# matthieugomez/LeastSquaresOptim.jl

Hardware: AMD Instinct MI355X
Metric: lm_lsmr_outer_iterations_per_sec (higher is better)
Workload: dtype f64

## Files before the change

leastsquaresoptim.jl_amd/csrc/lsq_optimize.hip:

```cpp
#include <chrono>
#include <cmath>
#include <cstring>

#include "lsq_solver.h"
#include "lsq_spmv.h"

static constexpr double MIN_DELTA = 1e-16, MAX_DELTA = 1e16, MIN_STEP_QUALITY = 1e-3;
static constexpr double MIN_DIAGONAL = 1e-6, MAX_DIAGONAL = 1e32;
static constexpr double DECREASE_THRESHOLD = 0.25, INCREASE_THRESHOLD = 0.75;

enum { SL_GRAD = 8, SL_DX = 9, SL_NONFIN = 10, SL_TRIAL = 11, SL_PRED = 12, SL_SSR = 13, SL_W0 = 14, SL_W1 = 15,
       SL_W2 = 16, SL_SUM = 17 };

extern "C" int lsq_solver_create(lsq_ctx *c, lsq_mat *J, int kind, int for_lm, lsq_solver **out) {
    LSQ_RANGE("lsq_solver_create");
    if (!c || !J || !out) return LSQ_EARG;
    if (kind == LSQ_QR && J->kind != LSQ_MAT_DENSE) {
        lsq_set_error("solver QR() is not available for sparse Jacobians. Choose between Cholesky() and LSMR()");
        return LSQ_EARG;
    }
    const bool blockdiag = kind == LSQ_CHOLESKY && J->kind == LSQ_MAT_CSC && J->bd_blocks > 0;
    const bool bordered = kind == LSQ_CHOLESKY && J->kind == LSQ_MAT_CSC && J->br_blocks > 0;
    if (kind == LSQ_CHOLESKY && J->kind != LSQ_MAT_DENSE && !blockdiag && !bordered) {
        lsq_set_error("MethodError: no AbstractAllocatedSolver for Cholesky() with a sparse Jacobian "
// ... 377 lines not shown
    }
}

static inline int ngrid(const lsq_ctx *c, long long n) {
    long long g = (n + LSQ_NT - 1) / LSQ_NT;
    long long cap = (long long)c->num_cus * 8;
    if (g > cap) g = cap;
    return g < 1 ? 1 : (int)g;
}

static int sumsq_to_slot(lsq_ctx *c, bool exact, long long n, const double *x, int ctr, double *d_out,
                         LsqSlotPublish pub = LsqSlotPublish()) {
    if (exact) return lsq_seq_reduce(c, 1, (int)n, x, nullptr, nullptr, d_out);
    long long g = (n + LSQ_NT - 1) / LSQ_NT, cap = (long long)c->num_cus * 2;
    if (g > cap) g = cap;
    if (g < 1) g = 1;
    LSQ_LAUNCH(k_sumsq_slot, dim3((int)g), dim3(LSQ_NT), 0, c->stream, n, x, c->d_partials, lsq_ctr(c, ctr), d_out,
                       pub);
    return LSQ_OK;
}
static int model_f(double *out, const double *x, void *user);
static int model_g(lsq_mat *J, const double *x, void *user);
static int model_f_sumsq(void *user, double *out, const double *x, int ctr, double *d_out, LsqSlotPublish pub, bool *done,
                         const int *skip = nullptr);
struct SpecGrad {
    int *gate;
    double ssr;
    double *grad;
    bool launched;
};
static int model_pair_tail(void *user, lsq_mat *J, const double *dx, const double *fcur, double *ftrial, const double *xt,
                           double *slot_pred, double *slot_trial, LsqSlotPublish pub, const int *skip, bool *done,
                           SpecGrad *sg = nullptr);
static void model_trial_buffers(void *user, const double *xt, double **t_out, double **s_out);
static int f_then_sumsq(lsq_ctx *c, bool exact, lsq_f_callback f, void *user, long long m, double *out, const double *x, int ctr,
                        double *d_out, LsqSlotPublish pub = LsqSlotPublish(), const int *skip = nullptr) {
    if (!exact && f == model_f) {
        bool fused = false;
        if (model_f_sumsq(user, out, x, ctr, d_out, pub, &fused, skip) != 0) {
            lsq_set_error("user callback reported failure");
            return LSQ_ECALLBACK;
        }
        if (fused) return LSQ_OK;
    } else if (f(out, x, user) != 0) {
        lsq_set_error("user callback reported failure");
        return LSQ_ECALLBACK;
    }
    return sumsq_to_slot(c, exact, m, out, ctr, d_out, pub);
}
static int predicted_to_slot(lsq_ctx *c, bool exact, lsq_mat *J, const double *d, const double *f, double *scratch,
                             int ctr, double *d_out, LsqSlotPublish pub = LsqSlotPublish(), const int *skip = nullptr);
static int wdot_to_slot(lsq_ctx *c, bool exact, int n, const double *x, const double *y, const double *w, int ctr,
                        double *d_out);
static int gradient_into(lsq_ctx *c, bool exact, lsq_mat *J, const double *f, double *g);

struct LoopBuffers {
    lsq_ctx *c;
    int m, n;
    double *dx = nullptr, *dtd = nullptr, *xt = nullptr, *ftrial = nullptr;
    double *dgn = nullptr, *dgr = nullptr, *grad = nullptr, *fpred = nullptr;
    double *lo = nullptr, *hi = nullptr;
    int *gate_ring = nullptr;
// ... 174 lines not shown
            return LSQ_ECALLBACK;                         \
        }                                                 \
    } while (0)

static int call_g(lsq_g_callback g, lsq_mat *J, const double *x, void *user) {
    J->version++;
    if (J->kind == LSQ_MAT_CSC && !J->d_cs_user) J->csr_fresh = false;
    CB(g(J, x, user));
    return lsq_ensure_csr(J);
}
int lsq_call_g(lsq_g_callback g, lsq_mat *J, const double *x, void *user) { return call_g(g, J, x, user); }

struct IterateGuard {
    lsq_ctx *c;
    double *&x, *&fcur;
    double *x_user, *fcur_user;
    int m, n;
    ~IterateGuard() {
        if (x != x_user) lsq_d2d(c, x_user, x, (size_t)n * sizeof(double));
        if (fcur != fcur_user) lsq_d2d(c, fcur_user, fcur, (size_t)m * sizeof(double));
    }
};

static int start_residual(lsq_ctx *c, lsq_mat *J, lsq_f_callback f, void *user, double *fcur, const double *x, double *ssr,
                          int *nonfinite_at) {
    const int m = J->m, n = J->n;
    if (lsq_small_mat(J) || lsq_small_vec(m) || m <= 0) {
        CB(f(fcur, x, user));
        LSQ_TRY(lsq_sumsq(c, m, fcur, ssr));
        return lsq_first_nonfinite(c, n, x, nonfinite_at);
    }
    static_assert(SL_TRIAL == SL_NONFIN + 1, "the two scalars of the loop head travel together");
    LSQ_TRY(lsq_first_nonfinite_to_slot(c, n, x, c->d_slots + SL_NONFIN));
    LSQ_TRY(f_then_sumsq(c, false, f, user, m, fcur, x, 7, c->d_slots + SL_TRIAL));
    double sl[2];
    LSQ_TRY(lsq_read_slots(c, SL_NONFIN, 2, sl));
    *nonfinite_at = (int)sl[0];
    *ssr = sl[1];
    return LSQ_OK;
}

static int optimize_lm_loop(lsq_ctx *c, lsq_solver *sv, LoopBuffers &b, lsq_mat *J, double *x_user, double *fcur_user,
                            lsq_f_callback f, lsq_g_callback g, void *user, const lsq_options *o, lsq_result *r);
static int optimize_lm(lsq_ctx *c, lsq_solver *sv, LoopBuffers &b, lsq_mat *J, double *x_user, double *fcur_user,
                       lsq_f_callback f, lsq_g_callback g, void *user, const lsq_options *o, lsq_result *r) {
    ShardedExit ex{c, o};
    return ex.finish(optimize_lm_loop(c, sv, b, J, x_user, fcur_user, f, g, user, o, r));
}
static int optimize_lm_loop(lsq_ctx *c, lsq_solver *sv, LoopBuffers &b, lsq_mat *J, double *x_user, double *fcur_user,
                            lsq_f_callback f, lsq_g_callback g, void *user, const lsq_options *o, lsq_result *r) {
    const int m = J->m, n = J->n;
    double *x = x_user, *fcur = fcur_user, *xt = b.xt, *ftrial = b.ftrial;
    IterateGuard guard{c, x, fcur, x_user, fcur_user, m, n};
    double delta = o->delta > 0 ? o->delta : 10.0;
    double decrease_factor = 2.0;
    int f_calls = 0, g_calls = 0, mul_calls = 0, xc = 0, fc = 0, gc = 0;
    bool converged = false;
    double ssr;
    int iter = 0, nonfinite_at = -1;
    const bool sharded = o->row_allreduce != nullptr;
    if (sharded) CB(f(fcur, x, user));
    else LSQ_TRY(start_residual(c, J, f, user, fcur, x, &ssr, &nonfinite_at));
    f_calls++;
    auto rows_sum = [&](double *d_buf, int count) -> int {
        if (o->row_allreduce(d_buf, count, (void *)c->stream, o->row_allreduce_user) != 0) {
            lsq_set_error("row all-reduce callback reported failure");
            return LSQ_ECALLBACK;
        }
        return LSQ_OK;
    };
    if (sharded) {
        LSQ_TRY(sumsq_to_slot(c, false, m, fcur, 7, c->d_slots + SL_TRIAL));
        LSQ_TRY(rows_sum(c->d_slots + SL_TRIAL, 1));
        LSQ_TRY(lsq_read_slots(c, SL_TRIAL, 1, &ssr));
        LSQ_TRY(lsq_first_nonfinite(c, n, x, &nonfinite_at));
    }
    r->ssr0 = ssr;
    double maxabs_gr = INFINITY;
    bool need_jac = true;
    const int gn = ngrid(c, n);
    const bool exact = lsq_small_mat(J) && !sharded && !(sv->kind == LSQ_LSMR && sv->gen_ldiv);
    int last_inner = 0;
    const bool no_spec_grad = getenv("LSQ_NO_SPEC_GRADIENT") != nullptr;
    bool spec_launched = false, spec_grad_ready = false, spec_pending = false;
    struct SpecGuard { lsq_mat *J; bool &ready; bool &pending; ~SpecGuard() { if (ready || pending) lsq_sparse_colsum_forget(J); } }
        spec_guard{J, spec_grad_ready, spec_pending};
    int local_done = 0;
    double gssr = ssr, ggr = maxabs_gr;
    long long inner_total = 0;
    while (iter < o->iterations) {
        if (!o->allreduce && converged) break;
        if (o->allreduce && converged) {
            int all = 1;
            gssr = ssr; ggr = maxabs_gr;
            LSQ_TRY(global_exchange(o, &gssr, &ggr, &all));
            if (all) break;
            ++iter; local_done = 1;
            continue;
        }
        iter++;
        if (nonfinite_at >= 0) {
            r->bad_index = nonfinite_at;
            r->iterations = iter - 1;
            lsq_set_error("IsFiniteException: non-finite x at index %d", nonfinite_at);
            return LSQ_ENONFINITE;
        }
        if (need_jac) {
            LSQ_TRY(call_g(g, J, x, user));
            g_calls++;
            need_jac = false;
        }
        bool have_grad = false;
        if (spec_grad_ready) {
            lsq_sparse_grad_colsum_adopt(J);
            have_grad = true;
            spec_grad_ready = false;
        }
        const bool spec_ok = !no_spec_grad && !exact && !sharded && sv->kind == LSQ_LSMR && f == model_f && g == model_g &&
                             iter < o->iterations && !lsq_dbg_serial;
        spec_launched = false;
        if (!exact && J->colsum_version != J->version && lsq_can_fuse_grad_colsum(J)) {
            LSQ_TRY(lsq_sparse_grad_colsum(J, fcur, b.grad));
            have_grad = true;
        }
        const double *cs = nullptr;
        LSQ_TRY(lsq_rowshard_colsum(sv, J, &cs));
        const bool one_wg = !exact && n <= LSQ_ONE_WG_N;
        const bool lm_prep = one_wg && sv->kind == LSQ_LSMR && ssr >= 0.0 && lsq_lsmr_takes_lm_prep(sv, J);
        if (exact) LSQ_TRY(lsq_exact_lm_damp(c, n, cs, 1.0 / delta, b.dtd));
        else if (!one_wg) LSQ_LAUNCH(k_lm_damp, dim3(1), dim3(1024), 0, c->stream, n, cs, 1.0 / delta, b.dtd);
        {
            if (!have_grad) LSQ_TRY(gradient_into(c, exact, J, fcur, b.grad));
            if (sharded) LSQ_TRY(rows_sum(b.grad, n));
            if (lm_prep) {}
            else if (one_wg)
// ... 1 lines not shown
                                   x, b.lo, b.hi, c->d_slots + SL_GRAD);
            else
                LSQ_LAUNCH(k_gradnorm, dim3(gn), dim3(LSQ_NT), 0, c->stream, n, b.grad, x, b.lo, b.hi,
                                   c->d_partials, lsq_ctr(c, 4), c->d_slots + SL_GRAD);
            mul_calls++;
        }
        struct Xchg { const lsq_options *o; double *gssr, *ggr; } xchg{o, &gssr, &ggr};
        if (o->allreduce) {
            gssr = ssr; ggr = maxabs_gr;
            c->idle_hook = [](void *p) -> int {
                Xchg *q = (Xchg *)p;
                int all = 0;
                return global_exchange(q->o, q->gssr, q->ggr, &all);
            };
            c->idle_user = &xchg;
            c->idle_status = 0;
            if (sv->kind != LSQ_LSMR || exact) lsq_run_idle_hook(c);
        }
        int lmiter = 0;
        struct TailCtx {
            lsq_ctx *c; lsq_mat *J; LoopBuffers *b; lsq_f_callback f; void *user;
            const double *x, *fcur; double *xt, *ftrial;
            int m, n, gn; bool is_model; LsqSlotPublish pub; int launched;
            bool want_spec; double ssr; bool spec_launched; bool *spec_pending;
        } tc{c, J, &b, f, user, x, fcur, xt, ftrial, m, n, gn, !exact && f == model_f, LsqSlotPublish(), 0, spec_ok, ssr, false,
             &spec_pending};
        auto tail_fn = [](const int *skip, void *u) -> int {
            TailCtx &t = *(TailCtx *)u;
            lsq_ctx *c = t.c;
            double *t_out = nullptr, *s_out = nullptr;
            if (t.is_model) model_trial_buffers(t.user, t.xt, &t_out, &s_out);
            LSQ_LAUNCH(k_step, dim3(t.gn), dim3(LSQ_NT), 0, c->stream, t.n, t.x, t.b->dx, t.xt, c->d_partials,
                               lsq_ctr(c, 5), c->d_slots + SL_DX, c->d_slots + SL_NONFIN, t_out, s_out, skip);
            LSQ_HIP(hipGetLastError());
            t.pub = lsq_slots_ticket(c, SL_GRAD, 6);
            bool pair = false;
            SpecGrad sg{t.want_spec ? next_gate(c, *t.b) : nullptr, t.ssr, t.b->grad, false};
            if (t.is_model && model_pair_tail(t.user, t.J, t.b->dx, t.fcur, t.ftrial, t.xt, c->d_slots + SL_PRED, c->d_slots + SL_TRIAL,
                                              t.pub, skip, &pair, &sg) != 0) {
                lsq_set_error("user callback reported failure");
                return LSQ_ECALLBACK;
            }
            t.spec_launched = sg.launched;
            if (sg.launched) *t.spec_pending = true;
            if (!pair) {
                LSQ_TRY(predicted_to_slot(c, false, t.J, t.b->dx, t.fcur, t.b->fpred, 8, c->d_slots + SL_PRED, LsqSlotPublish(), skip));
                LSQ_TRY(f_then_sumsq(c, false, t.f, t.user, t.m, t.ftrial, t.xt, 7, c->d_slots + SL_TRIAL, t.pub, skip));
            }
            LSQ_HIP(hipGetLastError());
            t.launched++;
            return LSQ_OK;
        };
        const bool tail_ok = !exact && !sharded && sv->kind == LSQ_LSMR && !b.lo && !b.hi;
        bool tail_done = false;
        if (sv->kind == LSQ_LSMR) {
            const LsmrLmPrep prep{cs, 1.0 / delta, MIN_DIAGONAL, MAX_DIAGONAL, x, b.lo, b.hi, c->d_slots + SL_GRAD};
            static const bool no_spec = getenv("LSQ_NO_TAIL_SPECULATION") != nullptr;
            const bool guardable = tc.is_model && J->kind == LSQ_MAT_CSC && J->srows.active && !no_spec && !lsq_dbg_serial;
            LsmrTail tail{guardable ? last_inner : 0, tail_fn, &tc, guardable};
            LSQ_TRY(lsq_lsmr_solve(sv, J, fcur, b.dtd, b.dx, &lmiter, b.grad, ssr, lm_prep ? &prep : nullptr,
// ... 27 lines not shown
                CB(f(ftrial, xt, user));
                f_calls++;
                LSQ_TRY(sumsq_to_slot(c, exact, m, ftrial, 7, c->d_slots + SL_TRIAL));
                LSQ_TRY(predicted_to_slot(c, exact, J, b.dx, fcur, b.fpred, 8, c->d_slots + SL_PRED));
                LSQ_HIP(hipGetLastError());
                LSQ_TRY(lsq_read_slots(c, SL_GRAD, 5, sl));
            } else {
                static_assert(SL_PRED == SL_TRIAL + 1, "trial and predicted ssr travel together");
                LSQ_TRY(predicted_to_slot(c, exact, J, b.dx, fcur, b.fpred, 8, c->d_slots + SL_PRED));
                LSQ_TRY(f_then_sumsq(c, exact, f, user, m, ftrial, xt, 7, c->d_slots + SL_TRIAL));
                f_calls++;
                LSQ_TRY(rows_sum(c->d_slots + SL_TRIAL, 2));
                LSQ_TRY(lsq_read_slots(c, SL_GRAD, 5, sl));
            }
        }
        mul_calls++;
        maxabs_gr = sl[0];
        const double maxabs_dx = sl[1];
        const int trial_nonfinite = (int)sl[2];
        const double trial_ssr = sl[3], predicted_ssr = sl[4];
        const double pred_red = std::fabs(ssr - predicted_ssr);
        const double rho = pred_red > 0 ? (ssr - trial_ssr) / pred_red : 0.0;
        const bool accepted = rho > MIN_STEP_QUALITY;
        const bool dev_accepted = spec_launched && sl[5] != 0.0;
        spec_grad_ready = spec_launched && accepted && dev_accepted;
        if (spec_launched && dev_accepted && !accepted) lsq_sparse_colsum_forget(J);
        spec_pending = false;
        converged = assess(maxabs_dx, maxabs_gr, ssr, trial_ssr, o->x_tol, o->f_tol, o->g_tol, accepted, &xc, &fc, &gc);
        if (accepted) {
            std::swap(fcur, ftrial);
            std::swap(x, xt);
            ssr = trial_ssr;
            double q = 1.0 - (2.0 * rho - 1.0) * (2.0 * rho - 1.0) * (2.0 * rho - 1.0);
            delta = std::min(delta / std::max(1.0 / 3.0, q), MAX_DELTA);
            decrease_factor = 2.0;
            need_jac = true;
            nonfinite_at = trial_nonfinite;
        } else {
            LSQ_LAUNCH(k_revert, dim3(gn), dim3(LSQ_NT), 0, c->stream, n, xt, b.dx, x);
            nonfinite_at = trial_nonfinite;
            delta = std::max(delta / decrease_factor, MIN_DELTA);
            decrease_factor *= 2.0;
        }
        record(o, c, iter, n, ssr, maxabs_gr, delta, rho, lmiter, accepted ? 1 : 0, x);
    }
    (void)local_done;
    LSQ_HIP(hipStreamSynchronize(c->stream));
    r->optimizer = LSQ_LEVENBERG_MARQUARDT;
    r->ssr = o->allreduce ? gssr : ssr;
    r->iterations = iter;
    r->converged = converged; r->x_converged = xc; r->f_converged = fc; r->g_converged = gc;
// ... 296 lines not shown
    double *partials;
    unsigned *counter;
    double *slot;
    LsqSlotPublish pub;
    __device__ void seg(int i, double dot, double &racc) const { seg_pre(i, dot, b[i], racc); }
    using has_pre = void;
    __device__ double pre(int i) const { return b[i]; }
    __device__ void seg_pre(int i, double dot, double bi, double &racc) const {
        const double v = dot - bi;
        out[i] = v;
        racc += v * v;
    }
    __device__ void extra(int, double &) const {}
    __device__ void finalize(double t) const {
        *slot = t;
        if (pub.count > 0) {
            for (int i = 0; i < pub.count; ++i)
                __hip_atomic_store(pub.dst + i, pub.src + i == slot ? t : pub.src[i], __ATOMIC_RELAXED, __HIP_MEMORY_SCOPE_SYSTEM);
            __hip_atomic_store(pub.seq_word, pub.seq, __ATOMIC_RELEASE, __HIP_MEMORY_SCOPE_SYSTEM);
        }
    }
};

__global__ void __launch_bounds__(LSQ_NT)
k_scale_cols(int n, const int *__restrict__ colptr, int m_dense, const double *__restrict__ A,
             const double *__restrict__ x, double *__restrict__ out) {
    for (int j = blockIdx.x; j < n; j += gridDim.x) {
        double t = tanh(x[j]);
        double s = 1.0 - t * t;
        long long k0 = colptr ? colptr[j] : (long long)j * m_dense;
        long long k1 = colptr ? colptr[j + 1] : (long long)(j + 1) * m_dense;
        for (long long k = k0 + threadIdx.x; k < k1; k += LSQ_NT) out[k] = A[k] * s;
    }
}
__global__ void __launch_bounds__(LSQ_NT)
k_scale_dense(int m, const double *__restrict__ A, const double *__restrict__ x, double *__restrict__ out) {
    const int j = blockIdx.x;
    const double t = tanh(x[j]);
    const double sfac = 1.0 - t * t;
    const size_t base = (size_t)j * m;
    for (int i = blockIdx.y * LSQ_NT + threadIdx.x; i < m; i += gridDim.y * LSQ_NT) out[base + i] = A[base + i] * sfac;
}
__global__ void __launch_bounds__(LSQ_NT)
k_scale_csr(long long nnz, const int *__restrict__ colidx, const double *__restrict__ A, const double *__restrict__ sfac,
            double *__restrict__ out) {
    for (long long k = blockIdx.x * (long long)LSQ_NT + threadIdx.x; k < nnz; k += (long long)gridDim.x * LSQ_NT)
        out[k] = A[k] * sfac[colidx[k]];
}
__global__ void __launch_bounds__(LSQ_NT) k_tanh_sfac(int n, const double *__restrict__ x, double *__restrict__ t,
                                                      double *__restrict__ s) {
    for (int i = blockIdx.x * LSQ_NT + threadIdx.x; i < n; i += gridDim.x * LSQ_NT) {
        const double v = tanh(x[i]);
        t[i] = v;
        s[i] = 1.0 - v * v;
    }
}
__global__ void __launch_bounds__(LSQ_NT) k_sfac(int n, const double *__restrict__ x, double *__restrict__ s) {
    for (int i = blockIdx.x * LSQ_NT + threadIdx.x; i < n; i += gridDim.x * LSQ_NT) {
        double t = tanh(x[i]);
        s[i] = 1.0 - t * t;
    }
}

__global__ void __launch_bounds__(LSQ_NT)
k_scale_bcsc(int nseg, int n, const int *__restrict__ ptr, const double *__restrict__ A, const double *__restrict__ sfac,
             double *__restrict__ out) {
    const int lane = threadIdx.x & 63, per = LSQ_NT / 64;
    for (int s = blockIdx.x * per + (threadIdx.x >> 6); s < nseg; s += gridDim.x * per) {
        const double f = sfac[s % n];
        const int k1 = ptr[s + 1];
        for (int k = ptr[s] + lane; k < k1; k += 64) out[k] = A[k] * f;
    }
}

typedef double lsq_d2 __attribute__((ext_vector_type(2)));
template <bool NT>
__global__ void __launch_bounds__(1024)
k_scale_lds(long long nnz4, const unsigned short *__restrict__ col16, const double *__restrict__ A,
// ... 47 lines not shown
        if (launch_sell_rows(J, nullptr, md->d_t, e, md->fused ? nullptr : md->d_Acsr) != LSQ_OK) return 1;
    } else if (J->kind == LSQ_MAT_CSC) {
        LsqSegs A = J->csr;
        A.d_val = md->d_Acsr;
        if (launch_segs<false>(c, A, md->d_t, e) != LSQ_OK) return 1;
    } else {
        lsq_mat tmp = *J;
        tmp.d_dense = md->d_Acsc;
        if (launch_product(&tmp, 0, md->d_t, e) != LSQ_OK) return 1;
    }
    return hipGetLastError() == hipSuccess ? 0 : 1;
}

static void model_trial_buffers(void *user, const double *xt, double **t_out, double **s_out) {
    lsq_model *md = (lsq_model *)user;
    md->tanh_x = md->sfac_x = nullptr;
    if ((md->J->kind == LSQ_MAT_CSC && md->J->srows.active) || md->J->kind == LSQ_MAT_DENSE) {
        *t_out = md->d_t;
        *s_out = md->d_sspec;
        md->tanh_x = md->sfac_x = xt;
    }
}

static int model_f_sumsq(void *user, double *out, const double *x, int ctr, double *d_out, LsqSlotPublish pub, bool *done,
                         const int *skip) {
    lsq_model *md = (lsq_model *)user;
    lsq_ctx *c = md->ctx;
    lsq_mat *J = md->J;
    *done = false;
    if (!(J->kind == LSQ_MAT_CSC && J->srows.active)) return model_f(out, x, user);
    model_perm_invalidate(md, out);
    EpiResidualSq e{skip, 0, md->d_b, out, c->d_partials, lsq_ctr(c, ctr), d_out, pub};
    const bool have_tanh = md->tanh_x == x;
    md->tanh_x = nullptr;
    if (!have_tanh) {
        md->sfac_x = nullptr;
        LSQ_LAUNCH(k_tanh, dim3(ngrid(c, J->n)), dim3(LSQ_NT), 0, c->stream, J->n, x, md->d_t);
    }
    if (launch_sell_rows(J, nullptr, md->d_t, e, md->fused ? nullptr : md->d_Acsr) != LSQ_OK) return 1;
    *done = true;
    return hipGetLastError() == hipSuccess ? 0 : 1;
}

static int model_pair_tail(void *user, lsq_mat *J, const double *dx, const double *fcur, double *ftrial, const double *xt,
                           double *slot_pred, double *slot_trial, LsqSlotPublish pub, const int *skip, bool *done, SpecGrad *sg) {
    lsq_model *md = (lsq_model *)user;
    lsq_ctx *c = md->ctx;
    *done = false;
    if (!(md->fused && J == md->J && J->kind == LSQ_MAT_CSC && J->srows.active && J->srows.ncw == 1 && J->d_colscale &&
          J->n <= LSQ_PAIR_X_MAX && md->tanh_x == xt) || getenv("LSQ_NO_PAIR_TAIL"))
        return 0;
    const LsqSell &S = J->srows;
    const int nxpad = (J->n + 1) & ~1;
    const size_t lds = (size_t)std::max(2 * nxpad, LSQ_SELL_ROWS_MAX) * sizeof(double);
    if (lsq_set_lds(c, (const void *)k_sell_rows_pair<0>, (size_t)2 * LSQ_PAIR_X_MAX * sizeof(double)) != LSQ_OK) return 0;
    const size_t plen = (size_t)S.nslices * 64;
    const int pgrid = std::max(1, std::min(lsq_div_up((long long)plen, LSQ_NT), c->num_cus * 8));
    if (!md->d_b_perm) {
        double *pb = nullptr, *p0 = nullptr, *p1 = nullptr;
        if (hipMalloc(&pb, plen * sizeof(double)) != hipSuccess || hipMalloc(&p0, plen * sizeof(double)) != hipSuccess ||
            hipMalloc(&p1, plen * sizeof(double)) != hipSuccess) {
            (void)hipGetLastError();
            hipFree(pb); hipFree(p0); hipFree(p1);
            return 0;
        }
        md->d_b_perm = pb; md->d_perm[0] = p0; md->d_perm[1] = p1;
        LSQ_LAUNCH(k_sell_perm_rows<0>, dim3(pgrid), dim3(LSQ_NT), 0, c->stream, sell_dev(S), S.wrows, S.nslices, (const double *)md->d_b,
                   md->d_b_perm);
    }
    int k = md->perm_of[0] == fcur ? 0 : (md->perm_of[1] == fcur ? 1 : -1);
    if (k < 0) {
        k = 0;
        LSQ_LAUNCH(k_sell_perm_rows<0>, dim3(pgrid), dim3(LSQ_NT), 0, c->stream, sell_dev(S), S.wrows, S.nslices, fcur, md->d_perm[k]);
        md->perm_of[k] = fcur;
    }
    md->perm_of[1 - k] = ftrial;
    md->tanh_x = nullptr;
    const int grid = std::max(1, std::min(S.nblocks, c->num_cus));
    const bool spec = sg && sg->gate && md->sfac_x == xt;
    SellPairEpi e{skip, md->d_perm[k], md->d_b_perm, ftrial, md->d_perm[1 - k], c->d_partials, c->d_partials + 4096, lsq_ctr(c, 7),
                  slot_pred, slot_trial, pub, spec ? sg->gate : nullptr, spec ? sg->ssr : 0.0, MIN_STEP_QUALITY,
                  c->d_slots + SL_SSR};
    LSQ_LAUNCH(k_sell_rows_pair<0>, dim3(grid), dim3(LSQ_BIG_NT), lds, c->stream, sell_dev(S), S.wrows, J->m, dx, J->d_colscale,
               (const double *)md->d_t, J->n, nxpad, e);
    *done = true;
    if (hipGetLastError() != hipSuccess) return 1;
    if (spec) {
        const int st = lsq_sparse_grad_colsum_spec(J, ftrial, sg->grad, md->d_sspec, sg->gate);
        if (st == LSQ_OK) sg->launched = true;
        else if (st != LSQ_EARG) return 1;
    }
    return 0;
}

static int model_g(lsq_mat *J, const double *x, void *user) {
    lsq_model *md = (lsq_model *)user;
    lsq_ctx *c = md->ctx;
    if (J->kind == LSQ_MAT_DENSE) {}
    else if (md->sfac_x == x) std::swap(md->d_s, md->d_sspec);
    else LSQ_LAUNCH(k_sfac, dim3(ngrid(c, J->n)), dim3(LSQ_NT), 0, c->stream, J->n, x, md->d_s);
    md->sfac_x = nullptr;
    md->tanh_x = nullptr;
    if (md->fused) {
        if (lsq_mat_set_colscale(J, md->d_s) != LSQ_OK) return 1;
        return hipGetLastError() == hipSuccess ? 0 : 1;
// ... 120 lines not shown
```

leastsquaresoptim.jl_amd/csrc/lsq_sell.h:

```cpp
#pragma once

constexpr int LSQ_SELL_POS_BITS = 13;
constexpr unsigned LSQ_SELL_POS_MASK = (1u << LSQ_SELL_POS_BITS) - 1u;
constexpr int LSQ_SELL_ROWS_MAX = 4096;
constexpr int LSQ_SELL_CW_AUTO = 6;
constexpr int LSQ_SELL_CW_MAX = 32;
constexpr int LSQ_SELL_GROWS_MAX = 16384;
constexpr int LSQ_SELL_CCOLS_MAX = 2560;

struct SellDev {
    const int2 *smeta;
    const unsigned *info;
    const unsigned short *idx16;
    const double *val;
    int nblocks;
    int spw;
};

template <int U>
struct SellBatch {
    double2 a[U];
    unsigned c[U];
};
template <int U, bool CLAMP>
// ... 82 lines not shown
    if (TAIL && (L & 1)) sell_tail_sum<SQ>(tail, L, len, xl, sum, sq);
}

template <bool SQ>
__device__ __forceinline__ void sell_lane_sum(const double *__restrict__ vp, const unsigned short *__restrict__ ip, int L, int len,
                                              const double *xl, double &sum, double &sq, int lane) {
    sell_lane_sum_from<SQ>(vp, ip, 0, L, len, xl, sum, sq, lane);
}

struct SellSliceRef {
    int2 sm;
    unsigned inf;
};
__device__ __forceinline__ SellSliceRef sell_slice_ref(const SellDev &S, int s, int s1, int lane) {
    SellSliceRef r;
    r.sm = make_int2(0, 0);
    r.inf = LSQ_SELL_POS_MASK;
    if (s < s1) {
        r.sm = S.smeta[__builtin_amdgcn_readfirstlane(s)];
        r.inf = S.info[(size_t)s * 64 + lane];
    }
    return r;
}
template <bool SQ, class Out>
__device__ __forceinline__ void sell_wave_slices(const SellDev &S, int s0, int s1, int wv, int lane, const double *xl, Out out) {
    constexpr int NW = LSQ_BIG_NT / 64;
    int s = s0 + wv;
    SellSliceRef A = sell_slice_ref(S, s, s1, lane);
    __syncthreads();
    for (; s < s1; s += NW) {
        const SellSliceRef a = A;
        A = sell_slice_ref(S, s + NW, s1, lane);
        const size_t oa = (size_t)a.sm.x + lane * 2;
        const unsigned pos = a.inf & LSQ_SELL_POS_MASK;
        double sum = 0.0, sq = 0.0;
        sell_lane_sum<SQ>(S.val + oa, S.idx16 + oa, a.sm.y, (int)(a.inf >> LSQ_SELL_POS_BITS), xl, sum, sq, lane);
        if (pos != LSQ_SELL_POS_MASK) out(pos, sum, sq);
    }
}

template <class Epi>
__global__ void __launch_bounds__(LSQ_BIG_NT) k_sell_rows(SellDev S, int wrows, int m, const double *__restrict__ x,
                                                          const double *__restrict__ xscale, int nx, int nxpad, Epi epi) {
    extern __shared__ __attribute__((aligned(16))) double smem[];
    __shared__ double sh[LSQ_BIG_NT / 64];
    double *xl = smem;
    double *yw = smem + nxpad;
    const int tid = threadIdx.x, lane = tid & 63, wv = tid >> 6;
    constexpr int XR = (LSQ_LDS_X_MAX + LSQ_BIG_NT - 1) / LSQ_BIG_NT;
    double xr[XR];
#pragma unroll
    for (int q = 0; q < XR; ++q) xr[q] = x[min(tid + q * LSQ_BIG_NT, nx - 1)];
    if (xscale) {
        double sr[XR];
#pragma unroll
        for (int q = 0; q < XR; ++q) sr[q] = xscale[min(tid + q * LSQ_BIG_NT, nx - 1)];
#pragma unroll
        for (int q = 0; q < XR; ++q) xr[q] *= sr[q];
    }
    const int dflag = epi.done ? *epi.done : 0;

    if constexpr (EpiHasBlockPrepare<Epi>::value) epi.block_prepare();
    if constexpr (EpiHasPrepare<Epi>::value) epi.prepare();
#pragma unroll
    for (int q = 0; q < XR; ++q)
        if (tid + q * LSQ_BIG_NT < nx) xl[tid + q * LSQ_BIG_NT] = xr[q];
    if (dflag) return;
    constexpr int Q = LSQ_SELL_ROWS_MAX / LSQ_BIG_NT;
    double racc = 0.0;
    for (int w = blockIdx.x; w < S.nblocks; w += gridDim.x) {
        const int base = w * wrows, rows = min(wrows, m - base);
        const int s0 = w * S.spw, s1 = s0 + S.spw;
        double pre[Q];
        if constexpr (EpiHasPre<Epi>::value) {
#pragma unroll
            for (int q = 0; q < Q; ++q) pre[q] = epi.pre(base + min(tid + q * LSQ_BIG_NT, rows - 1));
        }
        sell_wave_slices<false>(S, s0, s1, wv, lane, xl, [&](unsigned pos, double sum, double) { yw[pos] = sum; });
        __syncthreads();
#pragma unroll
        for (int q = 0; q < Q; ++q) {
            const int i = tid + q * LSQ_BIG_NT;
            if (i < rows) {
                if constexpr (EpiHasPre<Epi>::value) epi.seg_pre(base + i, yw[i], pre[q], racc);
                else epi.seg(base + i, yw[i], racc);
            }
        }
    }
    for (int e = blockIdx.x; e < epi.extra_blocks; e += gridDim.x)
        if (tid < LSQ_NT) epi.extra(e, racc);
    finish_block_nt<LSQ_BIG_NT>(epi, racc, sh);
}

template <int U, bool CLAMP>
__device__ __forceinline__ void sell_batch_sum2(SellBatch<U> &B, int p0, int np, int len, const double *xa, const double *xb,
                                                double &sa, double &sb) {
#pragma unroll
    for (int u = 0; u < U; ++u) {
        const unsigned i0 = B.c[u] & 0xffffu, i1 = B.c[u] >> 16;
        double a0 = B.a[u].x * xa[i0], a1 = B.a[u].y * xa[i1], b0 = B.a[u].x * xb[i0], b1 = B.a[u].y * xb[i1];
        asm volatile("" : "+v"(a0), "+v"(a1), "+v"(b0), "+v"(b1));
// ... 40 lines not shown
    if (L & 1) {
        double pa = tail.a * xa[tail.c], pb = tail.a * xb[tail.c];
        asm volatile("" : "+v"(pa), "+v"(pb));
        const bool in = L - 1 < len;
        const double ta = sa + pa, tb = sb + pb;
        sa = in ? ta : sa;
        sb = in ? tb : sb;
    }
}
constexpr int LSQ_PAIR_X_MAX = 10200;
struct SellPairEpi {
    const int *done;
    const double *fa;
    const double *fb;
    double *out_b;
    double *out_b_perm;
    double *part_a, *part_b;
    unsigned *counter;
    double *slot_a, *slot_b;
    LsqSlotPublish pub;
    int *gate;
    double ssr, min_quality;
    double *slot_gate;
};
template <int = 0>
__global__ void __launch_bounds__(LSQ_NT) k_sell_perm_rows(SellDev S, int wrows, int nslices, const double *__restrict__ src,
                                                           double *__restrict__ dst) {
    for (long long i = blockIdx.x * (long long)LSQ_NT + threadIdx.x; i < (long long)nslices * 64; i += (long long)gridDim.x * LSQ_NT) {
        const unsigned inf = S.info[i];
        const unsigned pos = inf & LSQ_SELL_POS_MASK;
        const int w = (int)(i >> 6) / S.spw;
        dst[i] = pos != LSQ_SELL_POS_MASK ? src[(size_t)w * wrows + pos] : 0.0;
    }
}
template <int = 0>
__global__ void __launch_bounds__(LSQ_BIG_NT) k_sell_rows_pair(SellDev S, int wrows, int m, const double *__restrict__ xa,
                                                               const double *__restrict__ sa_scale, const double *__restrict__ xb,
                                                               int nx, int nxpad, SellPairEpi e) {
    extern __shared__ __attribute__((aligned(16))) double smem[];
    __shared__ double sh[LSQ_BIG_NT / 64];
    double *la = smem, *lb = smem + nxpad;
    constexpr int NW = LSQ_BIG_NT / 64;
    const int tid = threadIdx.x, lane = tid & 63, wv = tid >> 6;
    constexpr int XR = (LSQ_PAIR_X_MAX + LSQ_BIG_NT - 1) / LSQ_BIG_NT;
    {
        double ra[XR], rs[XR], rb[XR];
// ... 58 lines not shown
        __syncthreads();
#pragma unroll
        for (int g = 0; g < G; ++g)
            if (kpos[g] != LSQ_SELL_POS_MASK) smem[kpos[g]] = keep[g];
        __syncthreads();
        for (int i = tid; i < rows; i += LSQ_BIG_NT) e.out_b[base + i] = smem[i];
    }
    const double ba = block_sum<LSQ_BIG_NT>(acc_a, sh);
    const double bb = block_sum<LSQ_BIG_NT>(acc_b, sh);
    if (tid == 0) __hip_atomic_store(&e.part_b[blockIdx.x], bb, RLX_AGENT);
    double total_a = 0.0;
    const bool last = grid_reduce<LSQ_BIG_NT>(ba, e.part_a, e.counter, gridDim.x, sh, [&](double t) { total_a = t; });
    if (!last) return;
    double pb = 0.0;
    for (int i = tid; i < (int)gridDim.x; i += LSQ_BIG_NT) pb += __hip_atomic_load(&e.part_b[i], RLX_AGENT);
    const double total_b = block_sum<LSQ_BIG_NT>(pb, sh);
    if (tid == 0) {
        *e.slot_a = total_a;
        *e.slot_b = total_b;
        if (e.gate) {
            const double pred_red = fabs(e.ssr - total_a);
            const double rho = pred_red > 0 ? (e.ssr - total_b) / pred_red : 0.0;
            const bool acc = rho > e.min_quality;
            *e.gate = acc ? 0 : 1;
            *e.slot_gate = acc ? 1.0 : 0.0;
        }
        if (e.pub.count > 0) {
            for (int i = 0; i < e.pub.count; ++i) {
                const double *src = e.pub.src + i;
                const double v = src == e.slot_a ? total_a : (src == e.slot_b ? total_b : *src);
                __hip_atomic_store(e.pub.dst + i, v, __ATOMIC_RELAXED, __HIP_MEMORY_SCOPE_SYSTEM);
            }
            __hip_atomic_store(e.pub.seq_word, e.pub.seq, __ATOMIC_RELEASE, __HIP_MEMORY_SCOPE_SYSTEM);
        }
    }
}

constexpr int LSQ_WIDE_NT = 512;
constexpr int LSQ_SELL_WIDE_X_MAX = 12544;
constexpr int LSQ_SELL_WIDE_G = LSQ_SELL_ROWS_MAX / 64 / (LSQ_WIDE_NT / 64);

template <class Epi>
__global__ void __launch_bounds__(LSQ_WIDE_NT) k_sell_rows_wide(SellDev S, int wrows, int m, int ncw, int cwidth,
                                                                const double *__restrict__ x, int nx, Epi epi) {
    extern __shared__ __attribute__((aligned(16))) double smem[];
    __shared__ double sh[LSQ_WIDE_NT / 64];
    constexpr int NW = LSQ_WIDE_NT / 64, G = LSQ_SELL_WIDE_G;
    double *xl = smem;
// ... 144 lines not shown
```

leastsquaresoptim.jl_amd/csrc/lsq_spmv.h:

```cpp
#pragma once
#include <hip/hip_ext.h>

#include <algorithm>
#include <type_traits>
#include <utility>

#include "lsq_common.h"

constexpr int LSQ_TILE_WINDOW = 2048;
constexpr int LSQ_TILE_NNZ = LSQ_TILE_WINDOW - 3;
constexpr int LSQ_TILE_SEGS = LSQ_NT;

struct SegsDev {
    const int *ptr;
    const int *idx;
    const double *val;
    const int *tiles;
    const unsigned short *idx16;
    int nseg;
    int ntiles;
    int nnz;
};


// ... 146 lines not shown
        const uint2 p = *reinterpret_cast<const uint2 *>(S.idx16 + k);
        return make_int4((int)(p.x & 0xffffu), (int)(p.x >> 16), (int)(p.y & 0xffffu), (int)(p.y >> 16));
    } else {
        return *reinterpret_cast<const int4 *>(S.idx + k);
    }
}

struct BigTileRegs {
    double2 v0[2], v1[2];
    int4 ci[2];
    int4 meta;
    int pa, pe;
    double pre;
};

template <class E, class = void>
struct EpiHasPrepare : std::false_type {};
template <class E>
struct EpiHasPrepare<E, std::void_t<typename E::has_prepare>> : std::true_type {};
template <class E, class = void>
struct EpiHasPre : std::false_type {};
template <class E>
struct EpiHasPre<E, std::void_t<typename E::has_pre>> : std::true_type {};

template <class Epi, bool IDX16>
__global__ void __launch_bounds__(LSQ_BIG_NT) k_seg_stream_lds(SegsDev S, const int4 *__restrict__ meta, int nbig,
                                                               const double *__restrict__ x, int nx, int nxpad,
                                                               Epi epi) {
    extern __shared__ __attribute__((aligned(16))) double smem[];
    __shared__ double sh[LSQ_BIG_NT / 64];
    double *xl = smem;
    double *prod = smem + nxpad;
    const int tid = threadIdx.x;
    const int G = gridDim.x;
    constexpr bool HAS_PRE = EpiHasPre<Epi>::value;
    const int kmax = (S.nnz + 3) & ~3;
    auto load_meta = [&](int tb) {
        int4 mt = meta[tb < nbig ? tb : nbig - 1];
        if (tb >= nbig) mt.y = mt.x;
        return mt;
    };
    auto load_data = [&](BigTileRegs &r, int4 mt) {
        r.meta = mt;
        const int ka = mt.z & ~3;
#pragma unroll
        for (int c = 0; c < 2; ++c) {
// ... 667 lines not shown
```

Baseline: 3976.

## Overlap start-up Jacobian with residual and fuse nonfinite check into tanh kernel

At the start of the LM loop, the nonfinite check is fused into the tanh/sfac kernel, and the residual is written directly in SELL-permuted order so the first pair tail can use it. The Jacobian evaluation and gradient colsum are launched before waiting on the host slot read, so they overlap the sync. The device-side speculative gate now also checks convergence, which stops speculative gradient work on the final iteration. This adds rollback paths (forgetting the cached point and colsum) for nonfinite or error cases, and makes the code more complex.

```diff
diff --git a/leastsquaresoptim.jl_amd/csrc/lsq_optimize.hip b/leastsquaresoptim.jl_amd/csrc/lsq_optimize.hip
--- a/leastsquaresoptim.jl_amd/csrc/lsq_optimize.hip
+++ b/leastsquaresoptim.jl_amd/csrc/lsq_optimize.hip
@@ -423,22 +423,25 @@
 static int model_f(double *out, const double *x, void *user);
 static int model_g(lsq_mat *J, const double *x, void *user);
 static int model_f_sumsq(void *user, double *out, const double *x, int ctr, double *d_out, LsqSlotPublish pub, bool *done,
-                         const int *skip = nullptr);
+                         const int *skip = nullptr, bool mirror = false);
+static int model_start_point(void *user, const double *x, double *d_nonfin, bool *done);
+static void model_forget_point(void *user);
 struct SpecGrad {
     int *gate;
     double ssr;
     double *grad;
     bool launched;
+    double xtol, ftol, gtol;
 };
 static int model_pair_tail(void *user, lsq_mat *J, const double *dx, const double *fcur, double *ftrial, const double *xt,
                            double *slot_pred, double *slot_trial, LsqSlotPublish pub, const int *skip, bool *done,
                            SpecGrad *sg = nullptr);
 static void model_trial_buffers(void *user, const double *xt, double **t_out, double **s_out);
 static int f_then_sumsq(lsq_ctx *c, bool exact, lsq_f_callback f, void *user, long long m, double *out, const double *x, int ctr,
-                        double *d_out, LsqSlotPublish pub = LsqSlotPublish(), const int *skip = nullptr) {
+                        double *d_out, LsqSlotPublish pub = LsqSlotPublish(), const int *skip = nullptr, bool mirror = false) {
     if (!exact && f == model_f) {
         bool fused = false;
-        if (model_f_sumsq(user, out, x, ctr, d_out, pub, &fused, skip) != 0) {
+        if (model_f_sumsq(user, out, x, ctr, d_out, pub, &fused, skip, mirror) != 0) {
             lsq_set_error("user callback reported failure");
             return LSQ_ECALLBACK;
         }
@@ -659,8 +662,12 @@
     }
 };
 
+struct StartAhead {
+    int (*fn)(void *);
+    void *user;
+};
 static int start_residual(lsq_ctx *c, lsq_mat *J, lsq_f_callback f, void *user, double *fcur, const double *x, double *ssr,
-                          int *nonfinite_at) {
+                          int *nonfinite_at, bool pair_next = false, const StartAhead *ahead = nullptr) {
     const int m = J->m, n = J->n;
     if (lsq_small_mat(J) || lsq_small_vec(m) || m <= 0) {
         CB(f(fcur, x, user));
@@ -668,10 +675,18 @@
         return lsq_first_nonfinite(c, n, x, nonfinite_at);
     }
     static_assert(SL_TRIAL == SL_NONFIN + 1, "the two scalars of the loop head travel together");
-    LSQ_TRY(lsq_first_nonfinite_to_slot(c, n, x, c->d_slots + SL_NONFIN));
-    LSQ_TRY(f_then_sumsq(c, false, f, user, m, fcur, x, 7, c->d_slots + SL_TRIAL));
+    bool head = false;
+    if (f == model_f && model_start_point(user, x, c->d_slots + SL_NONFIN, &head) != 0) return LSQ_EHIP;
+    if (!head) LSQ_TRY(lsq_first_nonfinite_to_slot(c, n, x, c->d_slots + SL_NONFIN));
+    const LsqSlotPublish pub = lsq_slots_ticket(c, SL_NONFIN, 2);
     double sl[2];
-    LSQ_TRY(lsq_read_slots(c, SL_NONFIN, 2, sl));
+    int st = f_then_sumsq(c, false, f, user, m, fcur, x, 7, c->d_slots + SL_TRIAL, pub, nullptr, pair_next);
+    if (st == LSQ_OK && head && ahead) st = ahead->fn(ahead->user);
+    if (st == LSQ_OK) st = lsq_wait_slots(c, SL_NONFIN, 2, pub.seq, sl);
+    if (st != LSQ_OK || (int)sl[0] >= 0) {
+        if (head) model_forget_point(user);
+        if (st != LSQ_OK) return st;
+    }
     *nonfinite_at = (int)sl[0];
     *ssr = sl[1];
     return LSQ_OK;
@@ -696,8 +711,27 @@
     double ssr;
     int iter = 0, nonfinite_at = -1;
     const bool sharded = o->row_allreduce != nullptr;
+    struct AheadCtx { lsq_g_callback g; lsq_mat *J; const double *x; void *user; const double *fcur; double *grad; bool g_done, grad_done; }
+        ah{g, J, x, user, fcur, b.grad, false, false};
+    const StartAhead ahead{[](void *p) -> int {
+        AheadCtx &a = *(AheadCtx *)p;
+        LSQ_TRY(call_g(a.g, a.J, a.x, a.user));
+        a.g_done = true;
+        if (a.J->colsum_version != a.J->version && lsq_can_fuse_grad_colsum(a.J)) {
+            LSQ_TRY(lsq_sparse_grad_colsum(a.J, a.fcur, a.grad));
+            a.grad_done = true;
+        }
+        return LSQ_OK;
+    }, &ah};
+    const bool ahead_ok = f == model_f && g == model_g && sv->kind == LSQ_LSMR && o->iterations > 0;
     if (sharded) CB(f(fcur, x, user));
-    else LSQ_TRY(start_residual(c, J, f, user, fcur, x, &ssr, &nonfinite_at));
+    else {
+        const int st = start_residual(c, J, f, user, fcur, x, &ssr, &nonfinite_at,
+                                      sv->kind == LSQ_LSMR && !o->h_lower && !o->h_upper && !lsq_small_mat(J),
+                                      ahead_ok ? &ahead : nullptr);
+        if (ah.g_done && (st != LSQ_OK || nonfinite_at >= 0)) lsq_sparse_colsum_forget(J);
+        LSQ_TRY(st);
+    }
     f_calls++;
     auto rows_sum = [&](double *d_buf, int count) -> int {
         if (o->row_allreduce(d_buf, count, (void *)c->stream, o->row_allreduce_user) != 0) {
@@ -743,11 +777,13 @@
             return LSQ_ENONFINITE;
         }
         if (need_jac) {
-            LSQ_TRY(call_g(g, J, x, user));
+            if (!ah.g_done) LSQ_TRY(call_g(g, J, x, user));
+            ah.g_done = false;
             g_calls++;
             need_jac = false;
         }
-        bool have_grad = false;
+        bool have_grad = ah.grad_done;
+        ah.grad_done = false;
         if (spec_grad_ready) {
             lsq_sparse_grad_colsum_adopt(J);
             have_grad = true;
@@ -795,9 +831,9 @@
             lsq_ctx *c; lsq_mat *J; LoopBuffers *b; lsq_f_callback f; void *user;
             const double *x, *fcur; double *xt, *ftrial;
             int m, n, gn; bool is_model; LsqSlotPublish pub; int launched;
-            bool want_spec; double ssr; bool spec_launched; bool *spec_pending;
+            bool want_spec; double ssr; bool spec_launched; bool *spec_pending; const lsq_options *o;
         } tc{c, J, &b, f, user, x, fcur, xt, ftrial, m, n, gn, !exact && f == model_f, LsqSlotPublish(), 0, spec_ok, ssr, false,
-             &spec_pending};
+             &spec_pending, o};
         auto tail_fn = [](const int *skip, void *u) -> int {
             TailCtx &t = *(TailCtx *)u;
             lsq_ctx *c = t.c;
@@ -808,7 +844,7 @@
             LSQ_HIP(hipGetLastError());
             t.pub = lsq_slots_ticket(c, SL_GRAD, 6);
             bool pair = false;
-            SpecGrad sg{t.want_spec ? next_gate(c, *t.b) : nullptr, t.ssr, t.b->grad, false};
+            SpecGrad sg{t.want_spec ? next_gate(c, *t.b) : nullptr, t.ssr, t.b->grad, false, t.o->x_tol, t.o->f_tol, t.o->g_tol};
             if (t.is_model && model_pair_tail(t.user, t.J, t.b->dx, t.fcur, t.ftrial, t.xt, c->d_slots + SL_PRED, c->d_slots + SL_TRIAL,
                                               t.pub, skip, &pair, &sg) != 0) {
                 lsq_set_error("user callback reported failure");
@@ -882,11 +918,12 @@
         const double pred_red = std::fabs(ssr - predicted_ssr);
         const double rho = pred_red > 0 ? (ssr - trial_ssr) / pred_red : 0.0;
         const bool accepted = rho > MIN_STEP_QUALITY;
-        const bool dev_accepted = spec_launched && sl[5] != 0.0;
-        spec_grad_ready = spec_launched && accepted && dev_accepted;
-        if (spec_launched && dev_accepted && !accepted) lsq_sparse_colsum_forget(J);
+        converged = assess(maxabs_dx, maxabs_gr, ssr, trial_ssr, o->x_tol, o->f_tol, o->g_tol, accepted, &xc, &fc, &gc);
+        const bool dev_ran = spec_launched && sl[5] != 0.0;
+        const bool host_goes_on = accepted && !converged;
+        spec_grad_ready = dev_ran && host_goes_on;
+        if (dev_ran && !host_goes_on) lsq_sparse_colsum_forget(J);
         spec_pending = false;
-        converged = assess(maxabs_dx, maxabs_gr, ssr, trial_ssr, o->x_tol, o->f_tol, o->g_tol, accepted, &xc, &fc, &gc);
         if (accepted) {
             std::swap(fcur, ftrial);
             std::swap(x, xt);
@@ -1229,6 +1266,14 @@
     }
 };
 
+struct EpiResidualSqPerm : EpiResidualSq {
+    const double *b_perm;
+    double *out_perm;
+    using has_slice_out = void;
+    __device__ double slice_pre(size_t pidx) const { return b_perm[pidx]; }
+    __device__ void slice_post(size_t pidx, double dot, double bi) const { out_perm[pidx] = dot - bi; }
+};
+
 __global__ void __launch_bounds__(LSQ_NT)
 k_scale_cols(int n, const int *__restrict__ colptr, int m_dense, const double *__restrict__ A,
              const double *__restrict__ x, double *__restrict__ out) {
@@ -1255,12 +1300,21 @@
         out[k] = A[k] * sfac[colidx[k]];
 }
 __global__ void __launch_bounds__(LSQ_NT) k_tanh_sfac(int n, const double *__restrict__ x, double *__restrict__ t,
-                                                      double *__restrict__ s) {
+                                                      double *__restrict__ s, double *partials, unsigned *counter,
+                                                      double *out_nonfin) {
+    __shared__ double sh[LSQ_NT / 64];
+    double code = 0.0;
     for (int i = blockIdx.x * LSQ_NT + threadIdx.x; i < n; i += gridDim.x * LSQ_NT) {
-        const double v = tanh(x[i]);
+        const double xi = x[i];
+        const double v = tanh(xi);
         t[i] = v;
         s[i] = 1.0 - v * v;
-    }
+        if (!isfinite(xi) && code == 0.0) code = 1e15 - (double)(i + 1);
+    }
+    const double bv = block_max<LSQ_NT>(code, sh);
+    grid_reduce<LSQ_NT, true>(bv, partials, counter, gridDim.x, sh, [=](double m) {
+        *out_nonfin = (m == 0.0) ? -1.0 : (1e15 - m) - 1.0;
+    });
 }
 __global__ void __launch_bounds__(LSQ_NT) k_sfac(int n, const double *__restrict__ x, double *__restrict__ s) {
     for (int i = blockIdx.x * LSQ_NT + threadIdx.x; i < n; i += gridDim.x * LSQ_NT) {
@@ -1354,8 +1408,50 @@
     }
 }
 
+static int model_start_point(void *user, const double *x, double *d_nonfin, bool *done) {
+    lsq_model *md = (lsq_model *)user;
+    lsq_ctx *c = md->ctx;
+    lsq_mat *J = md->J;
+    *done = false;
+    md->tanh_x = md->sfac_x = nullptr;
+    if (!(J->kind == LSQ_MAT_CSC && J->srows.active) || J->n <= 0) return 0;
+    LSQ_LAUNCH(k_tanh_sfac, dim3(ngrid(c, J->n)), dim3(LSQ_NT), 0, c->stream, J->n, x, md->d_t, md->d_sspec, c->d_partials,
+               lsq_ctr(c, 0), d_nonfin);
+    if (hipGetLastError() != hipSuccess) return 1;
+    md->tanh_x = md->sfac_x = x;
+    *done = true;
+    return 0;
+}
+static void model_forget_point(void *user) {
+    lsq_model *md = (lsq_model *)user;
+    md->tanh_x = md->sfac_x = nullptr;
+}
+
+static bool model_pair_applies(const lsq_model *md, const lsq_mat *J) {
+    return md->fused && J == md->J && J->kind == LSQ_MAT_CSC && J->srows.active && J->srows.ncw == 1 && J->d_colscale &&
+           J->n <= LSQ_PAIR_X_MAX && !getenv("LSQ_NO_PAIR_TAIL");
+}
+static bool model_perm_ready(lsq_model *md) {
+    if (md->d_b_perm) return true;
+    lsq_ctx *c = md->ctx;
+    const LsqSell &S = md->J->srows;
+    const size_t plen = (size_t)S.nslices * 64;
+    const int pgrid = std::max(1, std::min(lsq_div_up((long long)plen, LSQ_NT), c->num_cus * 8));
+    double *pb = nullptr, *p0 = nullptr, *p1 = nullptr;
+    if (hipMalloc(&pb, plen * sizeof(double)) != hipSuccess || hipMalloc(&p0, plen * sizeof(double)) != hipSuccess ||
+        hipMalloc(&p1, plen * sizeof(double)) != hipSuccess) {
+        (void)hipGetLastError();
+        hipFree(pb); hipFree(p0); hipFree(p1);
+        return false;
+    }
+    md->d_b_perm = pb; md->d_perm[0] = p0; md->d_perm[1] = p1;
+    LSQ_LAUNCH(k_sell_perm_rows<0>, dim3(pgrid), dim3(LSQ_NT), 0, c->stream, sell_dev(S), S.wrows, S.nslices, (const double *)md->d_b,
+               md->d_b_perm);
+    return true;
+}
+
 static int model_f_sumsq(void *user, double *out, const double *x, int ctr, double *d_out, LsqSlotPublish pub, bool *done,
-                         const int *skip) {
+                         const int *skip, bool mirror) {
     lsq_model *md = (lsq_model *)user;
     lsq_ctx *c = md->ctx;
     lsq_mat *J = md->J;
@@ -1369,7 +1465,14 @@
         md->sfac_x = nullptr;
         LSQ_LAUNCH(k_tanh, dim3(ngrid(c, J->n)), dim3(LSQ_NT), 0, c->stream, J->n, x, md->d_t);
     }
-    if (launch_sell_rows(J, nullptr, md->d_t, e, md->fused ? nullptr : md->d_Acsr) != LSQ_OK) return 1;
+    if (mirror && !skip && model_pair_applies(md, J) && model_perm_ready(md)) {
+        EpiResidualSqPerm ep;
+        static_cast<EpiResidualSq &>(ep) = e;
+        ep.b_perm = md->d_b_perm;
+        ep.out_perm = md->d_perm[0];
+        if (launch_sell_rows(J, nullptr, md->d_t, ep, nullptr) != LSQ_OK) return 1;
+        md->perm_of[0] = out;
+    } else if (launch_sell_rows(J, nullptr, md->d_t, e, md->fused ? nullptr : md->d_Acsr) != LSQ_OK) return 1;
     *done = true;
     return hipGetLastError() == hipSuccess ? 0 : 1;
 }
@@ -1379,27 +1482,14 @@
     lsq_model *md = (lsq_model *)user;
     lsq_ctx *c = md->ctx;
     *done = false;
-    if (!(md->fused && J == md->J && J->kind == LSQ_MAT_CSC && J->srows.active && J->srows.ncw == 1 && J->d_colscale &&
-          J->n <= LSQ_PAIR_X_MAX && md->tanh_x == xt) || getenv("LSQ_NO_PAIR_TAIL"))
-        return 0;
+    if (!(model_pair_applies(md, J) && md->tanh_x == xt)) return 0;
     const LsqSell &S = J->srows;
     const int nxpad = (J->n + 1) & ~1;
     const size_t lds = (size_t)std::max(2 * nxpad, LSQ_SELL_ROWS_MAX) * sizeof(double);
     if (lsq_set_lds(c, (const void *)k_sell_rows_pair<0>, (size_t)2 * LSQ_PAIR_X_MAX * sizeof(double)) != LSQ_OK) return 0;
     const size_t plen = (size_t)S.nslices * 64;
     const int pgrid = std::max(1, std::min(lsq_div_up((long long)plen, LSQ_NT), c->num_cus * 8));
-    if (!md->d_b_perm) {
-        double *pb = nullptr, *p0 = nullptr, *p1 = nullptr;
-        if (hipMalloc(&pb, plen * sizeof(double)) != hipSuccess || hipMalloc(&p0, plen * sizeof(double)) != hipSuccess ||
-            hipMalloc(&p1, plen * sizeof(double)) != hipSuccess) {
-            (void)hipGetLastError();
-            hipFree(pb); hipFree(p0); hipFree(p1);
-            return 0;
-        }
-        md->d_b_perm = pb; md->d_perm[0] = p0; md->d_perm[1] = p1;
-        LSQ_LAUNCH(k_sell_perm_rows<0>, dim3(pgrid), dim3(LSQ_NT), 0, c->stream, sell_dev(S), S.wrows, S.nslices, (const double *)md->d_b,
-                   md->d_b_perm);
-    }
+    if (!model_perm_ready(md)) return 0;
     int k = md->perm_of[0] == fcur ? 0 : (md->perm_of[1] == fcur ? 1 : -1);
     if (k < 0) {
         k = 0;
@@ -1412,7 +1502,8 @@
     const bool spec = sg && sg->gate && md->sfac_x == xt;
     SellPairEpi e{skip, md->d_perm[k], md->d_b_perm, ftrial, md->d_perm[1 - k], c->d_partials, c->d_partials + 4096, lsq_ctr(c, 7),
                   slot_pred, slot_trial, pub, spec ? sg->gate : nullptr, spec ? sg->ssr : 0.0, MIN_STEP_QUALITY,
-                  c->d_slots + SL_SSR};
+                  c->d_slots + SL_SSR, c->d_slots + SL_DX, c->d_slots + SL_GRAD, spec ? sg->xtol : 0.0, spec ? sg->ftol : 0.0,
+                  spec ? sg->gtol : 0.0};
     LSQ_LAUNCH(k_sell_rows_pair<0>, dim3(grid), dim3(LSQ_BIG_NT), lds, c->stream, sell_dev(S), S.wrows, J->m, dx, J->d_colscale,
                (const double *)md->d_t, J->n, nxpad, e);
     *done = true;
diff --git a/leastsquaresoptim.jl_amd/csrc/lsq_sell.h b/leastsquaresoptim.jl_amd/csrc/lsq_sell.h
--- a/leastsquaresoptim.jl_amd/csrc/lsq_sell.h
+++ b/leastsquaresoptim.jl_amd/csrc/lsq_sell.h
@@ -128,8 +128,13 @@
     }
     return r;
 }
-template <bool SQ, class Out>
-__device__ __forceinline__ void sell_wave_slices(const SellDev &S, int s0, int s1, int wv, int lane, const double *xl, Out out) {
+struct SellNoSliceHook {
+    __device__ __forceinline__ double pre(size_t) const { return 0.0; }
+    __device__ __forceinline__ void post(size_t, double, double) const {}
+};
+template <bool SQ, class Out, class Hook = SellNoSliceHook>
+__device__ __forceinline__ void sell_wave_slices(const SellDev &S, int s0, int s1, int wv, int lane, const double *xl, Out out,
+                                                 Hook hook = Hook()) {
     constexpr int NW = LSQ_BIG_NT / 64;
     int s = s0 + wv;
     SellSliceRef A = sell_slice_ref(S, s, s1, lane);
@@ -139,11 +144,22 @@
         A = sell_slice_ref(S, s + NW, s1, lane);
         const size_t oa = (size_t)a.sm.x + lane * 2;
         const unsigned pos = a.inf & LSQ_SELL_POS_MASK;
+        const size_t pidx = (size_t)s * 64 + lane;
+        const double hp = hook.pre(pidx);
         double sum = 0.0, sq = 0.0;
         sell_lane_sum<SQ>(S.val + oa, S.idx16 + oa, a.sm.y, (int)(a.inf >> LSQ_SELL_POS_BITS), xl, sum, sq, lane);
-        if (pos != LSQ_SELL_POS_MASK) out(pos, sum, sq);
-    }
-}
+        if (pos != LSQ_SELL_POS_MASK) {
+            out(pos, sum, sq);
+            hook.post(pidx, sum, hp);
+        }
+    }
+}
+template <class Epi>
+struct SellEpiSliceHook {
+    const Epi &epi;
+    __device__ __forceinline__ double pre(size_t pidx) const { return epi.slice_pre(pidx); }
+    __device__ __forceinline__ void post(size_t pidx, double sum, double p) const { epi.slice_post(pidx, sum, p); }
+};
 
 template <class Epi>
 __global__ void __launch_bounds__(LSQ_BIG_NT) k_sell_rows(SellDev S, int wrows, int m, const double *__restrict__ x,
@@ -182,7 +198,11 @@
 #pragma unroll
             for (int q = 0; q < Q; ++q) pre[q] = epi.pre(base + min(tid + q * LSQ_BIG_NT, rows - 1));
         }
-        sell_wave_slices<false>(S, s0, s1, wv, lane, xl, [&](unsigned pos, double sum, double) { yw[pos] = sum; });
+        if constexpr (EpiHasSliceOut<Epi>::value)
+            sell_wave_slices<false>(S, s0, s1, wv, lane, xl, [&](unsigned pos, double sum, double) { yw[pos] = sum; },
+                                    SellEpiSliceHook<Epi>{epi});
+        else
+            sell_wave_slices<false>(S, s0, s1, wv, lane, xl, [&](unsigned pos, double sum, double) { yw[pos] = sum; });
         __syncthreads();
 #pragma unroll
         for (int q = 0; q < Q; ++q) {
@@ -269,6 +289,8 @@
     int *gate;
     double ssr, min_quality;
     double *slot_gate;
+    const double *slot_dx, *slot_gr;
+    double xtol, ftol, gtol;
 };
 template <int = 0>
 __global__ void __launch_bounds__(LSQ_NT) k_sell_perm_rows(SellDev S, int wrows, int nslices, const double *__restrict__ src,
@@ -373,8 +395,11 @@
             const double pred_red = fabs(e.ssr - total_a);
             const double rho = pred_red > 0 ? (e.ssr - total_b) / pred_red : 0.0;
             const bool acc = rho > e.min_quality;
-            *e.gate = acc ? 0 : 1;
-            *e.slot_gate = acc ? 1.0 : 0.0;
+            const bool conv = (acc && fabs(total_b - e.ssr) <= e.ftol * (fabs(e.ssr) + e.ftol)) || *e.slot_dx <= e.xtol ||
+                              *e.slot_gr <= e.gtol;
+            const bool go = acc && !conv;
+            *e.gate = go ? 0 : 1;
+            *e.slot_gate = go ? 1.0 : 0.0;
         }
         if (e.pub.count > 0) {
             for (int i = 0; i < e.pub.count; ++i) {
diff --git a/leastsquaresoptim.jl_amd/csrc/lsq_spmv.h b/leastsquaresoptim.jl_amd/csrc/lsq_spmv.h
--- a/leastsquaresoptim.jl_amd/csrc/lsq_spmv.h
+++ b/leastsquaresoptim.jl_amd/csrc/lsq_spmv.h
@@ -192,6 +192,10 @@
 struct EpiHasPre : std::false_type {};
 template <class E>
 struct EpiHasPre<E, std::void_t<typename E::has_pre>> : std::true_type {};
+template <class E, class = void>
+struct EpiHasSliceOut : std::false_type {};
+template <class E>
+struct EpiHasSliceOut<E, std::void_t<typename E::has_slice_out>> : std::true_type {};
 
 template <class Epi, bool IDX16>
 __global__ void __launch_bounds__(LSQ_BIG_NT) k_seg_stream_lds(SegsDev S, const int4 *__restrict__ meta, int nbig,
```

After: 4088, median of 6. 1.03x the previous value.
